# ccuchengwei/LongReadSelfCorrect

Measured on NVIDIA B200. Metric: corrected Mbp/s (seed + FM-extend + DP/MSA fallback, default options), higher is better.
Workload: dtype int64+f64

## Files before the change

### longreadselfcorrect_b200/csrc/pbsc_dp.cu

```cuda
#include <cub/cub.cuh>
#include <stdio.h>
#include <stdlib.h>
#include <string.h>
#include <algorithm>
#include <vector>
#include <type_traits>
#include "pbsc_batch.cuh"
#include "pbsc_task.cuh"
#include <chrono>
#include "pbsc_dp.cuh"
#include "pbsc_dp_thread.cuh"
#include "pbsc_dp_msa.cuh"

namespace pbsc {

constexpr int DP_HALF = 100;
constexpr int DP_BW = 2 * DP_HALF + 1;
constexpr int DP_CPL = 7;
constexpr int DP_NEG = -(1 << 28);
constexpr int DP_WARPS = 8;

struct __align__(16) DpJob
{
    uint64_t lo[4];
// ... 201 lines not shown
    }
    int bestRowVal = 0, bestRowI = 0, bestColVal = 0, bestColJ = 0;
    bool anyRow = false, anyCol = false;
    #pragma unroll 1
    for (int i = 1; i <= qlen; i++)
    {
        const int jb = origin + i;
        const int first = max(jb, 1);
        const int last = min(jb + DP_BW, nRows) - 1;
        const bool skipCol = (last + 1 <= 0) || first >= nRows || first > last;
        const int rlo = skipCol ? (1 << 20) : first - jb, rhi = skipCol ? (1 << 20) : last - jb;
        const unsigned span = skipCol ? 0u : (unsigned)(rhi - rlo);
        const int rowNoLeft = (rhi != rlo) ? rhi : -1;
        const int c1 = (int)q[i - 1];
        const int pn0 = __shfl_down_sync(FULL, prev[0], 1);
        int a[DP_CPL], cur[DP_CPL];
        int run = DP_NEG;
        #pragma unroll
        for (int t = 0; t < DP_CPL; t++)
        {
            const int r = rbase + t;
            const bool comp = (unsigned)(r - rlo) <= span;
            const int sub = sw[t] == c1 ? 1 : -8;
            const int pl = (t < DP_CPL - 1) ? prev[t + 1] : pn0;
            const int left1 = (r != rowNoLeft) ? pl - 1 : DP_NEG;
            const int v0 = __viaddmax_s32(prev[t], sub, left1);
            run = comp ? __viaddmax_s32(v0, r, run) : run;
            a[t] = run;
        }
        int incl = run;
        #pragma unroll
        for (int off = 1; off < 32; off <<= 1)
        {
            const int o = __shfl_up_sync(FULL, incl, off);
            if (lane >= off) incl = max(incl, o);
        }
        int excl = __shfl_up_sync(FULL, incl, 1);
        if (lane == 0) excl = DP_NEG;
        #pragma unroll
        for (int t = 0; t < DP_CPL; t++)
        {
            const int r = rbase + t;
            const bool comp = (unsigned)(r - rlo) <= span;
            cur[t] = comp ? max(a[t], excl) - r : idle[t];
        }
        int upPrev = __shfl_up_sync(FULL, cur[DP_CPL - 1], 1);
        if (lane == 0) upPrev = DP_NEG;
        uint32_t w = 0;
        #pragma unroll
        for (int t = 0; t < DP_CPL; t++)
        {
            const int r = rbase + t;
            const bool comp = (unsigned)(r - rlo) <= span;
            const int diag = prev[t] + (sw[t] == c1 ? 1 : -8);
            const int pl = (t < DP_CPL - 1) ? prev[t + 1] : pn0;
            const int upv = t > 0 ? cur[t - 1] : upPrev;
            uint32_t f = (cur[t] == diag) ? 1u : 0u;
            f |= (cur[t] == upv - 1) ? 2u : 0u;
            f |= (cur[t] == pl - 1) ? 4u : 0u;
            w |= (comp ? f : 0u) << (3 * t);
        }
        flags[(size_t)i * 32 + lane] = w;
        if (!skipCol && last == nRows - 1)
        {
            const int vv = __shfl_sync(FULL, incl, 31) - rhi;
            if (!anyRow || vv > bestRowVal) { bestRowVal = vv; bestRowI = i; anyRow = true; }
        }
        if (i == qlen && !skipCol)
        {
            int lv = DP_NEG, lr = 0x7fffffff;
            #pragma unroll
            for (int t = 0; t < DP_CPL; t++)
            {
                const int r = rbase + t;
                const bool comp = (unsigned)(r - rlo) <= span;
                if (comp && cur[t] > lv) { lv = cur[t]; lr = r; }
            }
            #pragma unroll
            for (int off = 16; off > 0; off >>= 1)
            {
                const int ov = __shfl_xor_sync(FULL, lv, off), orr = __shfl_xor_sync(FULL, lr, off);
                if (ov > lv || (ov == lv && orr < lr)) { lv = ov; lr = orr; }
            }
            if (lr != 0x7fffffff) { anyCol = true; bestColVal = lv; bestColJ = jb + lr; }
        }
        const int nx = __shfl_down_sync(FULL, sw[0], 1);
        #pragma unroll
        for (int t = 0; t < DP_CPL; t++) { prev[t] = cur[t]; if (t < DP_CPL - 1) sw[t] = sw[t + 1]; }
        if (lane == 31)
        {
            const int j = jb + 1 + rbase + (DP_CPL - 1);
            sw[DP_CPL - 1] = (j >= 1 && j <= mlen) ? (int)s2[j - 1] : -1;
        }
        else sw[DP_CPL - 1] = nx;
    }
    if (anyCol && (!anyRow || bestColVal > bestRowVal)) { bi = qlen; bj = bestColJ; }
    else { bi = anyRow ? bestRowI : 0; bj = nRows - 1; }
    if (!(anyRow || anyCol) || bi <= 0 || bj <= 0) bi = 0;
}

#ifndef PBSC_DP_MINB
#define PBSC_DP_MINB 2
#endif
__global__ void __launch_bounds__(DP_WARPS * 32, PBSC_DP_MINB)
dp_align_kernel(uint64_t n_rows, DpRow* rows, const DpJob* __restrict__ jobs, const WalkTask* __restrict__ tasks, uint8_t* mem, uint64_t mem0,
                uint32_t* arenas, uint64_t arena_words, unsigned long long* counter, unsigned int* n_bad)
{
    const int lane = threadIdx.x & 31;
    const int wib = threadIdx.x >> 5;
    uint32_t* arena = arenas + ((size_t)blockIdx.x * DP_WARPS + wib) * arena_words;
    for (;;)
    {
        unsigned long long base = 0;
        if (lane == 0) base = atomicAdd(counter, 32ull);
        base = __shfl_sync(FULL, base, 0);
        if (base >= n_rows) break;
        const int nb = (int)min((unsigned long long)32, n_rows - base);
        int g0 = 0;
        uint64_t used = 0;
        uint64_t my_off = 0; int my_bi = 0, my_bj = 0; bool my_todo = false;
        for (int kk = 0; kk <= nb; kk++)
        {
            uint64_t need = 0;
            DpRow R; DpJob J; RowGeom g;
            bool fill = false;
            if (kk < nb)
            {
                R = rows[base + kk];
                if (R.pass == 2)
                {
                    J = jobs[R.job];
                    row_geometry(R, J, mem, mem0, g);
                    need = ((uint64_t)g.qlen + 1) * 32;
                    fill = true;
                }
            }
            if (kk == nb || (fill && used + need > arena_words))
            {
                __syncwarp();
                if (lane >= g0 && lane < kk && my_todo)
                {
                    DpRow Rm = rows[base + lane];
                    const DpJob Jm = jobs[Rm.job];
                    RowGeom gm;
                    row_geometry(Rm, Jm, mem, mem0, gm);
                    const uint32_t* fl = arena + my_off;
                    const uint8_t* __restrict__ s2 = gm.s2;
                    const uint8_t* __restrict__ q = gm.q;
                    const int qlen = gm.qlen, mlen = gm.mlen, origin = gm.origin;
                    int i = my_bi, j = my_bj, n = 0, ed = 0;
                    if (i <= 0) { atomicAdd(n_bad, 1u); Rm.pass = 0; }
                    else
                    {
                        int r = j - (origin + i);
                        uint32_t word = fl[(size_t)i * 32 + r / DP_CPL];
                        int wcol = i, widx = r / DP_CPL;
                        #pragma unroll 1
                        while (i > 0 && j > 0)
                        {
                            r = j - (origin + i);
                            const int wi = r / DP_CPL;
                            if (wcol != i || widx != wi) { word = fl[(size_t)i * 32 + wi]; wcol = i; widx = wi; }
                            const uint32_t nextWord = i > 1 ? fl[(size_t)(i - 1) * 32 + wi] : 0u;
                            const uint32_t f = (word >> (3 * (r - wi * DP_CPL))) & 7u;
                            const int s2p = (int)s2[j - 1], s2n = j < mlen ? (int)s2[j] : -1;
                            const int s1p = (int)q[i - 1], s1n = i < qlen ? (int)q[i] : -2;
                            const bool eqD = f & 1u, eqU = (f & 2u) != 0, eqL = (f & 4u) != 0;
                            int op;
                            if (s2p == s2n) op = eqU ? OP_I : (eqL ? OP_D : OP_M);
                            else if (s1p == s1n) op = eqL ? OP_D : (eqU ? OP_I : OP_M);
                            else op = eqD ? OP_M : (eqL ? OP_D : OP_I);
                            if (op == OP_M) { if (s1p != s2p) ed++; i--; j--; }
                            else if (op == OP_I) { ed++; j--; }
                            else { ed++; i--; }
                            if (op != OP_I) { word = nextWord; wcol = i; }
                            gm.ops[n] = (uint8_t)op;
                            n++;
                        }
                        const WalkTask& tk = tasks[Jm.task];
                        const uint64_t fsum = (uint64_t)(int64_t)tk.freq_sum;
                        double identity = 0.65;
                        identity = __dadd_rn(identity, fsum > 50 ? 0.05 : 0.0);
                        identity = __dadd_rn(identity, fsum > 100 ? 0.05 : 0.0);
                        const double pct = __ddiv_rn(__dmul_rn((double)(n - ed), 100.0), (double)n);
                        const bool passOverlap = (uint64_t)n >= (uint64_t)(qlen / 10);
                        const bool passIdentity = __ddiv_rn(pct, 100.0) >= identity;
                        Rm.nops = (uint32_t)n; Rm.start0 = i; Rm.start1 = j;
                        Rm.pass = (passOverlap && passIdentity) ? 1u : 0u;
                    }
                    rows[base + lane] = Rm;
                    my_todo = false;
                }
                __syncwarp();
                g0 = kk; used = 0;
            }
            if (fill)
            {
                int bi, bj;
                dp_fill_row(g, arena + used, bi, bj);
                if (lane == kk) { my_off = used; my_bi = bi; my_bj = bj; my_todo = true; }
                used += need;
            }
        }
    }
}

template <int QMAX_, int NT_, bool GREAD_>
struct DptCfg
{
    static constexpr int QMAX = QMAX_;
    static constexpr int NT = NT_;
    static constexpr bool GREAD = GREAD_;
    static constexpr int HWORDS = dpt::HSLOTS / 2;
    static constexpr int SWORDS = (dpt::max_len_bound(QMAX_) + 15) / 16 + 1;
    static constexpr int SMEM = (HWORDS + (GREAD_ ? 0 : SWORDS)) * NT_ * 4;
};
using DptShort = DptCfg<256, 128, false>;
using DptLong = DptCfg<1024, 64, true>;
using DptHuge = DptCfg<4000, 32, true>;
constexpr uint32_t DPT_KEY_NONE = 0x3FFFu;
constexpr int DPT_KEY_BITS = 14;

__device__ __forceinline__ int dp_row_origin(const DpRow& R, const DpJob& J)
{
    const int k = (int)J.k, qlen = (int)J.qlen, mlen = (int)R.len;
    const bool isRC = R.local >= J.cnt[0] + J.cnt[1];
    const int start_1 = isRC ? qlen - k : 0, start_2 = isRC ? mlen - k : 0;
    return (start_2 - start_1 + 1) - (DP_HALF + 1);
}

__global__ void __launch_bounds__(256)
dp_keys_kernel(uint64_t n_rows, const DpRow* __restrict__ rows, const DpJob* __restrict__ jobs, uint32_t* keys, uint32_t* order, int qmax,
               unsigned long long* n_eligible)
{
    const uint64_t i = blockIdx.x * (uint64_t)blockDim.x + threadIdx.x;
    if (i >= n_rows) return;
    const DpRow R = rows[i];
    uint32_t key = DPT_KEY_NONE;
    if (R.pass == 2)
    {
        const DpJob J = jobs[R.job];
        if (dpt::eligible((int)J.qlen, (int)R.len, dp_row_origin(R, J), qmax))
            key = ((uint32_t)(qmax - (int)J.qlen) << 1) | (R.local >= J.cnt[0] + J.cnt[1] ? 1u : 0u);
    }
    keys[i] = key;
    order[i] = (uint32_t)i;
    const unsigned m = __ballot_sync(__activemask(), key != DPT_KEY_NONE);
    if (key != DPT_KEY_NONE && (threadIdx.x & 31) == __ffs(m) - 1) atomicAdd(n_eligible, (unsigned long long)__popc(m));
}

template <class C>
struct DptH
{
    uint32_t* p;
    __device__ __forceinline__ int get(int j) const
    {
        const int s = j & (dpt::HSLOTS - 1);
        return (int)reinterpret_cast<const short*>(p + (s >> 1) * C::NT)[s & 1];
    }
    __device__ __forceinline__ void set(int j, int v)
    {
        const int s = j & (dpt::HSLOTS - 1);
        reinterpret_cast<short*>(p + (s >> 1) * C::NT)[s & 1] = (short)v;
    }
    __device__ __forceinline__ bool pairs_ok(int j) const { return ((j >> 1) & (C::HWORDS - 1)) <= C::HWORDS - 5; }
    __device__ __forceinline__ uint32_t get2(int j, int u) const { return p[((j >> 1) & (C::HWORDS - 1)) * C::NT + u * C::NT]; }
    __device__ __forceinline__ void set2(int j, int u, uint32_t w) { p[((j >> 1) & (C::HWORDS - 1)) * C::NT + u * C::NT] = w; }
};
template <class C>
struct DptS
{
    const uint32_t* p;
    __device__ __forceinline__ int base(int x) const { return (int)((p[(x >> 4) * C::NT] >> (2 * (x & 15))) & 3u); }
    __device__ __forceinline__ uint32_t bits(int x) const
    {
        const uint32_t* w = p + (x >> 4) * C::NT;
        return __funnelshift_r(w[0], w[C::NT], 2 * (x & 15));
    }
};
struct DptSG
{
    const uint32_t* p;
    __device__ __forceinline__ int base(int x) const { return (int)((p[(size_t)(x >> 4) * 32] >> (2 * (x & 15))) & 3u); }
    __device__ __forceinline__ uint32_t bits(int x) const
    {
        const uint32_t* w = p + (size_t)(x >> 4) * 32;
        return __funnelshift_r(w[0], w[32], 2 * (x & 15));
    }
};
struct DptF
{
    uint32_t* p;
    __device__ __forceinline__ void put(int n, uint32_t w) { p[(size_t)n * 32] = w; }
    __device__ __forceinline__ uint32_t get(int n) const { return p[(size_t)n * 32]; }
};
struct DptQ { const uint8_t* q; __device__ __forceinline__ int operator()(int x) const { return (int)q[x]; } };
struct DptOps { uint8_t* ops; __device__ __forceinline__ void put(int n, int op) { ops[n] = (uint8_t)op; } };

template <class C>
__global__ void __launch_bounds__(C::NT, 227 * 1024 / (C::SMEM + 1024))
dp_align_thread_kernel(uint64_t n_rows, const uint32_t* __restrict__ keys, const uint32_t* __restrict__ order, DpRow* rows,
                       const DpJob* __restrict__ jobs, const WalkTask* __restrict__ tasks, uint8_t* mem, uint64_t mem0, uint32_t* arenas,
                       uint64_t arena_words, unsigned long long* counter, unsigned int* n_bad, const unsigned long long* __restrict__ n_eligible,
                       unsigned long long min_rows, unsigned int* n_thread_rows, uint32_t* rarena)
{
    extern __shared__ uint32_t dpt_smem[];
    const unsigned long long n_el = *n_eligible;
    if (n_el < min_rows) return;
    if (blockIdx.x == 0 && threadIdx.x == 0) atomicAdd(n_thread_rows, (unsigned int)n_el);
    const int lane = threadIdx.x & 31;
    uint32_t* Hs = dpt_smem + threadIdx.x;
    const uint64_t warp = (uint64_t)blockIdx.x * (C::NT / 32) + (threadIdx.x >> 5);
    uint32_t* Ss = C::GREAD ? rarena + warp * (uint64_t)(C::SWORDS * 32) + lane : dpt_smem + C::HWORDS * C::NT + threadIdx.x;
    constexpr int SSTRIDE = C::GREAD ? 32 : C::NT;
    DptF F{arenas + warp * arena_words + lane};
    for (;;)
    {
        unsigned long long base = 0;
        if (lane == 0) base = atomicAdd(counter, 32ull);
        base = __shfl_sync(FULL, base, 0);
        if (base >= n_rows) break;
        const uint64_t t = base + lane;
        const uint32_t key = t < n_rows ? keys[t] : DPT_KEY_NONE;
        if (__shfl_sync(FULL, key, 0) == DPT_KEY_NONE) break;
        if (key == DPT_KEY_NONE) continue;
        const uint64_t ri = order[t];
        DpRow R = rows[ri];
        const DpJob J = jobs[R.job];
        RowGeom g;
        row_geometry(R, J, mem, mem0, g);
        for (int x = 0; x < g.mlen; x += 16)
        {
            uint32_t w = 0;
            const int m = min(16, g.mlen - x);
            for (int y = 0; y < m; y++) w |= (uint32_t)g.s2[x + y] << (2 * y);
            Ss[(x >> 4) * SSTRIDE] = w;
        }
        Ss[((g.mlen + 15) >> 4) * SSTRIDE] = 0u;
        #pragma unroll 8
        for (int x = 0; x < C::HWORDS; x++) Hs[x * C::NT] = 0u;
        DptH<C> H{Hs};
        const typename std::conditional<C::GREAD, DptSG, DptS<C>>::type S{Ss};
        const DptQ q{g.q};
        int bi, bj;
        dpt::fill(g.qlen, g.mlen, g.origin, H, S, F, q, bi, bj);
        if (bi <= 0) { atomicAdd(n_bad, 1u); R.pass = 0; }
        else
        {
            DptOps ops{g.ops};
            int n, ed, i0, j0;
            dpt::traceback(g.qlen, g.mlen, g.origin, S, F, q, bi, bj, ops, n, ed, i0, j0);
            const WalkTask& tk = tasks[J.task];
            const uint64_t fsum = (uint64_t)(int64_t)tk.freq_sum;
            double identity = 0.65;
            identity = __dadd_rn(identity, fsum > 50 ? 0.05 : 0.0);
            identity = __dadd_rn(identity, fsum > 100 ? 0.05 : 0.0);
            const double pct = __ddiv_rn(__dmul_rn((double)(n - ed), 100.0), (double)n);
            const bool passOverlap = (uint64_t)n >= (uint64_t)(g.qlen / 10);
            const bool passIdentity = __ddiv_rn(pct, 100.0) >= identity;
            R.nops = (uint32_t)n; R.start0 = i0; R.start1 = j0;
            R.pass = (passOverlap && passIdentity) ? 1u : 0u;
        }
        rows[ri] = R;
    }
}

struct MsaCtx
{
    WalkTask& tk; uint8_t* outpool;
    __device__ __forceinline__ int min_call() const
    {
        const uint64_t fsum = (uint64_t)(int64_t)tk.freq_sum;
        return (int)(fsum > 50 ? (uint64_t)__dmul_rn((double)fsum, 0.4) : 15);
    }
    __device__ __forceinline__ uint8_t* out() const { return outpool + tk.out_off; }
    __device__ __forceinline__ uint32_t cap() const { return tk.out_cap; }
};

__global__ void __launch_bounds__(128)
dp_job_keys_kernel(uint64_t j0, uint64_t j1, const DpJob* __restrict__ jobs, const DpRow* __restrict__ rows, uint64_t row_base, uint32_t* keys,
                   uint32_t* order)
{
    const uint64_t t = blockIdx.x * (uint64_t)blockDim.x + threadIdx.x;
    if (j0 + t >= j1) return;
    const DpJob J = jobs[j0 + t];
    const uint32_t nr = job_rows_of(J);
    const DpRow* R = rows + (J.row0 - row_base);
    uint32_t passing = 0, cost = 0;
    for (uint32_t r = 0; r < nr; r++)
    {
        const DpRow x = R[r];
        if (x.pass == 1) { passing++; cost += x.nops; }
    }
    if (passing < 3) cost = 0;
    keys[t] = 0xFFFFu - min(0xFFFFu, cost >> 3);
    order[t] = (uint32_t)t;
}

__global__ void __launch_bounds__(64)
dp_msa_kernel(uint64_t j0, uint64_t j1, const uint32_t* __restrict__ order, int deal, const DpJob* __restrict__ jobs, WalkTask* tasks,
              const DpRow* __restrict__ rows, uint64_t row_base, uint8_t* mem, uint64_t mem0, uint8_t* outpool, unsigned int* n_bad,
              uint32_t big_thr, uint32_t* big_list, unsigned int* n_big)
{
    const uint64_t tx = blockIdx.x * (uint64_t)blockDim.x + threadIdx.x;
    const uint64_t njc = j1 - j0;
    uint64_t rank = tx;
    if (order && deal)
    {
        const uint64_t n_warps = (njc + 31) / 32;
        rank = (tx & 31) * n_warps + (tx >> 5);
        if (tx >= n_warps * 32) return;
    }
    if (rank >= njc) return;
    const uint64_t jx = j0 + (order ? order[rank] : rank);
    const DpJob J = jobs[jx];
    WalkTask& tk = tasks[J.task];
    const uint32_t nr = job_rows_of(J);
    const DpRow* R = rows + (J.row0 - row_base);
    if (big_list)
    {
        uint32_t cost = 0, passing = 0;
        for (uint32_t r = 0; r < nr; r++) { const DpRow x = R[r]; if (x.pass == 1) { passing++; cost += x.nops; } }
        if (passing >= 3 && cost >= big_thr) { big_list[atomicAdd(n_big, 1u)] = (uint32_t)(jx - j0); return; }
    }
    JobView v;
    job_view(mem + (J.mem - mem0), J, nr, v);
    const MsaCtx ctx{tk, outpool};
    uint32_t n = 0;
    const int rc = msa::consensus(v, J.qlen, J.k, R, nr, ctx, n);
    if (rc == 1) { tk.dp_status = PBSC_DP_FEW_ROWS; return; }
    if (rc == 2) { atomicAdd(n_bad, 1u); tk.dp_status = PBSC_OVF_DP; return; }
    tk.out_len = n;
    tk.dp_status = PBSC_DP_OK;
}

constexpr int MSA_WARPS = 4;
__global__ void __launch_bounds__(MSA_WARPS * 32)
dp_msa_warp_kernel(uint64_t j0, const uint32_t* __restrict__ big_list, const unsigned int* __restrict__ n_big, unsigned long long* counter,
                   const DpJob* __restrict__ jobs, WalkTask* tasks, const DpRow* __restrict__ rows, uint64_t row_base, uint8_t* mem, uint64_t mem0,
                   uint8_t* outpool, unsigned int* n_bad)
{
    __shared__ unsigned int gap_counter[MSA_WARPS];
    const int lane = threadIdx.x & 31, warp = threadIdx.x >> 5;
    const unsigned long long n = *n_big;
    for (;;)
    {
        unsigned long long it = 0;
        if (lane == 0) it = atomicAdd(counter, 1ull);
        it = __shfl_sync(0xffffffffu, it, 0);
        if (it >= n) break;
        const uint64_t jx = j0 + big_list[it];
        const DpJob J = jobs[jx];
        WalkTask& tk = tasks[J.task];
        const uint32_t nr = job_rows_of(J);
        const DpRow* R = rows + (J.row0 - row_base);
        JobView v;
        job_view(mem + (J.mem - mem0), J, nr, v);
        const MsaCtx ctx{tk, outpool};
        uint32_t nout = 0;
        const int rc = msa::consensus_warp(v, J.qlen, J.k, R, nr, ctx, nout, &gap_counter[warp]);
        __syncwarp();
        if (lane == 0)
        {
            if (rc == 1) tk.dp_status = PBSC_DP_FEW_ROWS;
            else if (rc == 2) { atomicAdd(n_bad, 1u); tk.dp_status = PBSC_OVF_DP; }
            else { tk.out_len = nout; tk.dp_status = PBSC_DP_OK; }
        }
        __syncwarp();
    }
}

template <class T>
static cudaError_t arena(pbsc_index* idx, const char* name, size_t count, T** out) { return arena_get(idx, name, (count ? count : 1) * sizeof(T), (void**)out); }

DpStats& last_dp_stats() { static thread_local DpStats s; return s; }

struct DptPass
{
    bool on = false; uint64_t qmax = 0, arena_words = 0, min_rows = 0, read_words = 0; int blocks = 0;
    uint64_t flag_words() const { return on ? arena_words * (uint64_t)blocks : 0; }
};
template <class C>
static cudaError_t dpt_pass_setup(pbsc_index* idx, uint64_t q_longest, uint64_t q_prev_max, int cap_per_sm, DptPass& g)
{
    g.on = q_longest > q_prev_max;
    if (!g.on) return cudaSuccess;
    g.qmax = std::min<uint64_t>((uint64_t)C::QMAX, q_longest);
    g.arena_words = 32ull * g.qmax * dpt::WMAX;
    cudaError_t e = cudaFuncSetAttribute(dp_align_thread_kernel<C>, cudaFuncAttributeMaxDynamicSharedMemorySize, C::SMEM);
    if (e != cudaSuccess) return e;
    int per = 0;
    e = cudaOccupancyMaxActiveBlocksPerMultiprocessor(&per, dp_align_thread_kernel<C>, C::NT, C::SMEM);
    if (e != cudaSuccess) return e;
    if (cap_per_sm > 0) per = std::min(per, cap_per_sm);
    g.blocks = idx->sm_count * std::max(per, 1);
    g.arena_words *= (uint64_t)(C::NT / 32);
    g.read_words = C::GREAD ? (uint64_t)g.blocks * (C::NT / 32) * (uint64_t)(C::SWORDS * 32) : 0;
    return cudaSuccess;
}
template <class C>
static void dpt_pass_launch(const DptPass& g, cudaStream_t st, uint64_t nrows, DpRow* rows, const DpJob* jobs, const WalkTask* tasks, uint8_t* mem,
                            uint64_t mem0, uint32_t* keys, uint32_t* keys2, uint32_t* order, uint32_t* order2, uint8_t* sort_tmp, size_t sort_bytes,
                            uint32_t* slabs, unsigned long long* counter, unsigned int* cnt, uint32_t* rarena)
{
    cudaMemsetAsync(counter, 0, 16, st);
    dp_keys_kernel<<<(unsigned)((nrows + 255) / 256), 256, 0, st>>>(nrows, rows, jobs, keys, order, (int)g.qmax, counter + 1);
    cub::DeviceRadixSort::SortPairs(sort_tmp, sort_bytes, keys, keys2, order, order2, (int)nrows, 0, DPT_KEY_BITS, st);
    const int tb = (int)std::min<uint64_t>((uint64_t)g.blocks, (nrows + C::NT - 1) / C::NT);
    dp_align_thread_kernel<C><<<tb, C::NT, C::SMEM, st>>>(nrows, keys2, order2, rows, jobs, tasks, mem, mem0, slabs, g.arena_words / (C::NT / 32), counter,
                                                          cnt + 1, counter + 1, g.min_rows, cnt + 2, rarena);
}

int run_dp_fallback(pbsc_index* idx, const pbsc_params* p, DeviceBatch& b, void* tasks_v, uint64_t n_items, const uint32_t* list, uint8_t* outpool,
                    uint32_t q_cap, uint64_t* launches)
{
    WalkTask* tasks = (WalkTask*)tasks_v;
    cudaStream_t st = idx->stream;
    if (n_items == 0) return PBSC_OK;
    const bool htrace = getenv("PBSC_ROUND_TRACE") != nullptr;
    auto h0 = std::chrono::steady_clock::now();
    auto hmark = [&](const char* what) {
        if (!htrace) return;
        const auto now = std::chrono::steady_clock::now();
        const double ms = std::chrono::duration<double, std::milli>(now - h0).count();
        if (ms > 2.0) fprintf(stderr, "[pbsc round trace]     dp host: %-22s %8.2f ms\n", what, ms);
        h0 = now;
    };
    DpJob* jobs; uint64_t *job_rows, *job_bytes, *row_off, *mem_off; unsigned int* cnt; unsigned long long* qctr;
    PBSC_CUDA(arena(idx, "dp.jobs", n_items, &jobs));
    PBSC_CUDA(arena(idx, "dp.job_rows", n_items + 1, &job_rows));
    PBSC_CUDA(arena(idx, "dp.job_bytes", n_items + 1, &job_bytes));
    PBSC_CUDA(arena(idx, "dp.row_off", n_items + 1, &row_off));
    PBSC_CUDA(arena(idx, "dp.mem_off", n_items + 1, &mem_off));
    PBSC_CUDA(arena(idx, "dp.cnt", 4, &cnt));
    PBSC_CUDA(arena(idx, "dp.qctr", 4, &qctr));
    PBSC_CUDA(cudaMemsetAsync(cnt, 0, 16, st));
    cudaEvent_t ev[2];
    PBSC_CUDA(cudaEventCreate(&ev[0])); PBSC_CUDA(cudaEventCreate(&ev[1]));
    struct EvGuard { cudaEvent_t* e; ~EvGuard() { cudaEventDestroy(e[0]); cudaEventDestroy(e[1]); } } guard{ev};
    PBSC_CUDA(cudaEventRecord(ev[0], st));
    dp_collect_kernel<<<(unsigned)((n_items + 127) / 128), 128, 0, st>>>(idx->dev, n_items, list, tasks, b.codes.p, b.offsets.p, (uint32_t)p->pb_coverage,
                                                                        jobs, job_rows, job_bytes, cnt);
    unsigned int hcnt[4] = {0, 0, 0, 0};
    PBSC_CUDA(cudaMemcpyAsync(hcnt, cnt, 16, cudaMemcpyDeviceToHost, st));
    PBSC_CUDA(cudaStreamSynchronize(st));
    if (launches) *launches += 1;
    const uint64_t nj = hcnt[0];
    DpStats& S = last_dp_stats();
    hmark("collect + sync");
    if (nj == 0) return PBSC_OK;
    {
        size_t tb = 0, tb2 = 0;
        cub::DeviceScan::ExclusiveSum(nullptr, tb, job_rows, row_off, (int)(nj + 1), st);
        cub::DeviceScan::ExclusiveSum(nullptr, tb2, job_bytes, mem_off, (int)(nj + 1), st);
        tb = std::max(tb, tb2);
        uint8_t* tmp;
        PBSC_CUDA(arena(idx, "dp.cubtmp", tb, &tmp));
        PBSC_CUDA(cudaMemsetAsync(job_rows + nj, 0, 8, st));
        PBSC_CUDA(cudaMemsetAsync(job_bytes + nj, 0, 8, st));
        cub::DeviceScan::ExclusiveSum(tmp, tb, job_rows, row_off, (int)(nj + 1), st);
        cub::DeviceScan::ExclusiveSum(tmp, tb, job_bytes, mem_off, (int)(nj + 1), st);
        dp_offsets_kernel<<<(unsigned)((nj + 255) / 256), 256, 0, st>>>(nj, jobs, row_off, mem_off);
    }
    std::vector<uint64_t> h_row(nj + 1), h_mem(nj + 1);
    PBSC_CUDA(cudaMemcpyAsync(h_row.data(), row_off, (nj + 1) * 8, cudaMemcpyDeviceToHost, st));
    PBSC_CUDA(cudaMemcpyAsync(h_mem.data(), mem_off, (nj + 1) * 8, cudaMemcpyDeviceToHost, st));
    PBSC_CUDA(cudaStreamSynchronize(st));
    if (launches) *launches += 3;
    hmark("scans + sync");
    S.jobs += nj; S.rows += h_row[nj];
    uint64_t budget = 20ull << 30;
    {
        const auto it = idx->arena.find("dp.mem");
        const uint64_t have = it != idx->arena.end() ? (uint64_t)it->second.cap : 0;
        if (h_mem[nj] > have)
        {
            size_t free_b = 0, total_b = 0;
            if (cudaMemGetInfo(&free_b, &total_b) == cudaSuccess) budget = std::min<uint64_t>(budget, std::max<uint64_t>(2ull << 30, (free_b + have) / 2));
        }
        else budget = std::max<uint64_t>(have, 1);
    }
    if (const char* e = getenv("PBSC_DP_CHUNK_MB")) { if (atoll(e) > 0) budget = (uint64_t)atoll(e) << 20; }
    uint64_t max_job = 0;
    for (uint64_t j = 0; j < nj; j++) max_job = std::max(max_job, h_mem[j + 1] - h_mem[j]);
    if (max_job > budget) budget = max_job;
    const uint64_t pool_bytes = std::min(budget, h_mem[nj]);
    uint8_t* mem;
    hmark("budget");
    PBSC_CUDA(arena(idx, "dp.mem", pool_bytes, &mem));
    hmark("arena dp.mem");
    int per_sm = 0;
    PBSC_CUDA(cudaOccupancyMaxActiveBlocksPerMultiprocessor(&per_sm, dp_align_kernel, DP_WARPS * 32, 0));
    if (per_sm < 1) per_sm = 1;
    if (const char* e = getenv("PBSC_DP_BLOCKS_PER_SM")) { if (atoi(e) > 0) per_sm = std::min(per_sm, atoi(e)); }
    const int ablocks = idx->sm_count * per_sm;
    uint64_t arena_words = std::max<uint64_t>(((uint64_t)q_cap + 2) * 32, 1ull << 18);
    if (const char* e = getenv("PBSC_DP_ARENA_KB")) { if (atoll(e) > 0) arena_words = std::max<uint64_t>(((uint64_t)q_cap + 2) * 32, (uint64_t)atoll(e) * 256); }
    uint32_t* slabs;
    PBSC_CUDA(arena(idx, "dp.flags", arena_words * (uint64_t)ablocks * DP_WARPS, &slabs));
    uint64_t max_rows = 0;
    for (uint64_t j0 = 0; j0 < nj;)
    {
        uint64_t j1 = j0 + 1;
        while (j1 < nj && h_mem[j1 + 1] - h_mem[j0] <= pool_bytes) j1++;
        max_rows = std::max(max_rows, h_row[j1] - h_row[j0]);
        j0 = j1;
    }
    DpRow* rows;
    hmark("flags arena + chunking");
    PBSC_CUDA(arena(idx, "dp.rows", max_rows, &rows));
    bool use_thread = true;
    if (const char* e = getenv("PBSC_DP_THREAD")) use_thread = atoi(e) != 0;
    uint32_t *tkeys = nullptr, *tkeys2 = nullptr, *torder = nullptr, *torder2 = nullptr, *tslabs = nullptr, *treads = nullptr;
    uint8_t* sort_tmp = nullptr;
    size_t sort_bytes = 0;
    const uint64_t q_longest = std::min<uint64_t>(q_cap, hcnt[3]);
    DptPass pass_s, pass_l, pass_h;
    if (use_thread)
    {
        int cap = 0;
        if (const char* e = getenv("PBSC_DPT_BLOCKS_PER_SM")) cap = atoi(e);
        const bool longer = !(getenv("PBSC_DPT_LONG") && atoi(getenv("PBSC_DPT_LONG")) == 0);
        PBSC_CUDA(dpt_pass_setup<DptShort>(idx, q_longest, 0, cap, pass_s));
        if (longer) PBSC_CUDA(dpt_pass_setup<DptLong>(idx, q_longest, DptShort::QMAX, 0, pass_l));
        if (longer) PBSC_CUDA(dpt_pass_setup<DptHuge>(idx, q_longest, DptLong::QMAX, 0, pass_h));
        pass_s.min_rows = 512; pass_l.min_rows = 2048; pass_h.min_rows = 2048;
        if (const char* e = getenv("PBSC_DPT_MIN_ROWS")) pass_s.min_rows = pass_l.min_rows = pass_h.min_rows = (uint64_t)std::max(0ll, atoll(e));
        PBSC_CUDA(arena(idx, "dp.tkeys", max_rows, &tkeys));
        PBSC_CUDA(arena(idx, "dp.tkeys2", max_rows, &tkeys2));
        PBSC_CUDA(arena(idx, "dp.torder", max_rows, &torder));
        PBSC_CUDA(arena(idx, "dp.torder2", max_rows, &torder2));
        cub::DeviceRadixSort::SortPairs(nullptr, sort_bytes, tkeys, tkeys2, torder, torder2, (int)max_rows, 0, DPT_KEY_BITS, st);
        PBSC_CUDA(arena(idx, "dp.sorttmp", sort_bytes, &sort_tmp));
        PBSC_CUDA(arena(idx, "dp.tflags", std::max(pass_s.flag_words(), std::max(pass_l.flag_words(), pass_h.flag_words())), &tslabs));
        PBSC_CUDA(arena(idx, "dp.treads", std::max<uint64_t>(1, std::max(pass_l.on ? pass_l.read_words : 0, pass_h.on ? pass_h.read_words : 0)), &treads));
    }
    int sort_jobs = 0;
    if (const char* e = getenv("PBSC_DP_SORT_JOBS")) sort_jobs = atoi(e);
    uint32_t *jkeys = nullptr, *jkeys2 = nullptr, *jord = nullptr, *jord2 = nullptr;
    uint8_t* jsort_tmp = nullptr;
    size_t jsort_bytes = 0;
    if (sort_jobs)
    {
        PBSC_CUDA(arena(idx, "dp.jkeys", nj, &jkeys));
        PBSC_CUDA(arena(idx, "dp.jkeys2", nj, &jkeys2));
        PBSC_CUDA(arena(idx, "dp.jord", nj, &jord));
        PBSC_CUDA(arena(idx, "dp.jord2", nj, &jord2));
        cub::DeviceRadixSort::SortPairs(nullptr, jsort_bytes, jkeys, jkeys2, jord, jord2, (int)nj, 0, 16, st);
        PBSC_CUDA(arena(idx, "dp.jsorttmp", jsort_bytes, &jsort_tmp));
    }
    uint32_t msa_big_thr = 8192;
    if (const char* e = getenv("PBSC_MSA_WARP_MIN")) msa_big_thr = atoll(e) < 0 ? 0xffffffffu : (uint32_t)atoll(e);
    uint32_t* msa_big = nullptr;
    unsigned long long* msa_q = nullptr;
    PBSC_CUDA(arena(idx, "dp.msa_big", nj, &msa_big));
    PBSC_CUDA(arena(idx, "dp.msa_q", 2, &msa_q));
    struct Prof
    {
        bool on = false; cudaStream_t st; std::vector<std::pair<const char*, cudaEvent_t>> ev;
        void mark(const char* name) { if (!on) return; cudaEvent_t e; cudaEventCreate(&e); cudaEventRecord(e, st); ev.emplace_back(name, e); }
        void report()
        {
            if (!on || ev.size() < 2) return;
            cudaEventSynchronize(ev.back().second);
            std::vector<std::pair<const char*, float>> acc;
            for (size_t x = 1; x < ev.size(); x++)
            {
                float ms = 0; cudaEventElapsedTime(&ms, ev[x - 1].second, ev[x].second);
                bool found = false;
                for (auto& a : acc) if (!strcmp(a.first, ev[x].first)) { a.second += ms; found = true; }
                if (!found) acc.emplace_back(ev[x].first, ms);
            }
            fprintf(stderr, "[pbsc dp profile]");
            for (auto& a : acc) fprintf(stderr, " %s %.1f ms;", a.first, a.second);
            fprintf(stderr, "\n");
            for (auto& e : ev) cudaEventDestroy(e.second);
        }
    } prof;
    prof.st = st;
    if (const char* e = getenv("PBSC_DP_PROFILE")) prof.on = atoi(e) != 0;
    hmark("pass setup + arenas");
    prof.mark("start");
    for (uint64_t j0 = 0; j0 < nj;)
    {
        uint64_t j1 = j0 + 1;
        while (j1 < nj && h_mem[j1 + 1] - h_mem[j0] <= pool_bytes) j1++;
        const uint64_t nrows = h_row[j1] - h_row[j0], njc = j1 - j0;
        dp_rows_kernel<<<(unsigned)((njc + 127) / 128), 128, 0, st>>>(j0, j1, jobs, tasks, b.codes.p, b.offsets.p, mem, h_mem[j0], rows, h_row[j0]);
        dp_retrieve_kernel<<<(unsigned)((nrows + 127) / 128), 128, 0, st>>>(idx->dev, nrows, rows, jobs, mem, h_mem[j0]);
        prof.mark("rows+retrieve");
        PBSC_CUDA(cudaMemsetAsync(qctr, 0, 32, st));
        if (pass_s.on)
        {
            dpt_pass_launch<DptShort>(pass_s, st, nrows, rows, jobs, tasks, mem, h_mem[j0], tkeys, tkeys2, torder, torder2, sort_tmp, sort_bytes, tslabs,
                                      qctr + 1, cnt, treads);
            prof.mark("align_thread_256");
            if (launches) *launches += 4;
        }
        if (pass_l.on)
        {
            dpt_pass_launch<DptLong>(pass_l, st, nrows, rows, jobs, tasks, mem, h_mem[j0], tkeys, tkeys2, torder, torder2, sort_tmp, sort_bytes, tslabs,
                                     qctr + 1, cnt, treads);
            prof.mark("align_thread_1024");
            if (launches) *launches += 4;
        }
        if (pass_h.on)
        {
            dpt_pass_launch<DptHuge>(pass_h, st, nrows, rows, jobs, tasks, mem, h_mem[j0], tkeys, tkeys2, torder, torder2, sort_tmp, sort_bytes, tslabs,
                                     qctr + 1, cnt, treads);
            prof.mark("align_thread_4000");
            if (launches) *launches += 4;
        }
        const int nb = (int)std::min<uint64_t>((uint64_t)ablocks, (nrows + DP_WARPS * 32 - 1) / (DP_WARPS * 32));
        dp_align_kernel<<<nb, DP_WARPS * 32, 0, st>>>(nrows, rows, jobs, tasks, mem, h_mem[j0], slabs, arena_words, qctr, cnt + 1);
        prof.mark("align_warp");
        const uint32_t* jorder = nullptr;
        if (sort_jobs)
        {
            dp_job_keys_kernel<<<(unsigned)((njc + 127) / 128), 128, 0, st>>>(j0, j1, jobs, rows, h_row[j0], jkeys, jord);
            size_t sb = jsort_bytes;
            cub::DeviceRadixSort::SortPairs(jsort_tmp, sb, jkeys, jkeys2, jord, jord2, (int)njc, 0, 16, st);
            jorder = jord2;
            if (launches) *launches += 3;
        }
        PBSC_CUDA(cudaMemsetAsync(msa_q, 0, 16, st));
        dp_msa_kernel<<<(unsigned)((((njc + 31) / 32) * 32 + 63) / 64), 64, 0, st>>>(j0, j1, jorder, sort_jobs == 1, jobs, tasks, rows, h_row[j0], mem,
                                                                                         h_mem[j0], outpool, cnt + 1, msa_big_thr,
                                                                                         msa_big_thr != 0xffffffffu ? msa_big : nullptr, (unsigned int*)(msa_q + 1));
        prof.mark("msa");
        if (msa_big_thr != 0xffffffffu)
        {
            const int wb = (int)std::min<uint64_t>((uint64_t)idx->sm_count * 4, (njc + MSA_WARPS - 1) / MSA_WARPS);
            dp_msa_warp_kernel<<<wb, MSA_WARPS * 32, 0, st>>>(j0, msa_big, (const unsigned int*)(msa_q + 1), msa_q, jobs, tasks, rows, h_row[j0], mem, h_mem[j0],
                                                              outpool, cnt + 1);
            prof.mark("msa_warp");
            if (launches) *launches += 1;
        }
        PBSC_CUDA(cudaGetLastError());
        if (launches) *launches += 4;
        S.chunks++;
        j0 = j1;
    }
    PBSC_CUDA(cudaEventRecord(ev[1], st));
    hmark("chunk loop (launches)");
    prof.report();
    PBSC_CUDA(cudaMemcpyAsync(hcnt, cnt, 12, cudaMemcpyDeviceToHost, st));
    PBSC_CUDA(cudaStreamSynchronize(st));
    S.bad += hcnt[1];
    S.thread_rows += hcnt[2];
    PBSC_OCC_TAKE(3, st);
    float ms = 0;
    cudaEventElapsedTime(&ms, ev[0], ev[1]);
    S.ms += ms;
    return PBSC_OK;
}

}
```

### longreadselfcorrect_b200/csrc/pbsc_dp_thread.cuh

```cuda
#ifndef PBSC_DP_THREAD_CUH
#define PBSC_DP_THREAD_CUH

#include <stdint.h>

#if defined(__CUDACC__)
#define PBSC_DPT_HD __host__ __device__ __forceinline__
#else
#define PBSC_DPT_HD inline
#endif

namespace pbsc { namespace dpt {

constexpr int HALF = 100;
constexpr int BW = 2 * HALF + 1;
constexpr int CPW = 10;
constexpr int WMAX = (BW + CPW - 1) / CPW;
constexpr int NEVER = -(1 << 28);
constexpr int OP_M = 0, OP_I = 1, OP_D = 2;
constexpr int HSLOTS = 256;

PBSC_DPT_HD uint32_t push_ne(uint32_t w, int v, int x)
{
#if defined(__CUDA_ARCH__)
    return __funnelshift_l((uint32_t)(x - v), w, 1);
#else
    return (w << 1) | ((uint32_t)(x - v) >> 31);
#endif
}
PBSC_DPT_HD int imax(int a, int b) { return a > b ? a : b; }
PBSC_DPT_HD int imin(int a, int b) { return a < b ? a : b; }

PBSC_DPT_HD constexpr int max_len_bound(int qmax) { return qmax + qmax / 10 + 21; }

PBSC_DPT_HD bool eligible(int qlen, int mlen, int , int qmax) { return qlen >= 1 && qlen <= qmax && mlen >= 1 && mlen <= max_len_bound(qmax); }
PBSC_DPT_HD int words_per_col(int mlen) { return (imin(BW, mlen) + 1 + CPW - 1) / CPW; }

template <class HS, class SS, class FS, class QF>
PBSC_DPT_HD void fill(int qlen, int mlen, int origin, HS& H, const SS& S, FS& F, const QF& q, int& bi, int& bj)
{
    const int nRows = mlen + 1;
    const int W = words_per_col(mlen);
    int bestRowVal = 0, bestRowI = 0;
    bool anyRow = false;
    int wbase = 0;
#if defined(__CUDA_ARCH__)
    #pragma unroll 1
#endif
    for (int i = 1; i <= qlen; i++, wbase += W)
    {
        const int jb = origin + i;
        const int first = imax(jb, 1);
        const int last = imin(jb + BW, nRows) - 1;
        if (last < first) continue;
        const int c1 = q(i - 1);
        const uint32_t c1rep = (uint32_t)c1 * 0x55555u;
        int j = first;
        int diagOld = H.get(j - 1);
        int widx = wbase, kin = (first & 1) + 1;
        int up, v;
        uint32_t w;
        {
            const int leftOld = H.get(j);
            const int d = diagOld + (S.base(j - 1) == c1 ? 1 : -8);
            const int l1 = (j == jb + BW - 1) ? NEVER : leftOld - 1;
            const int u1 = first > jb ? -1 : NEVER;
            v = imax(d, l1);
            w = (v == d ? 1u : 0u) | (v == u1 ? 2u : 0u) | (v == l1 ? 4u : 0u);
            H.set(j, v);
            up = v; diagOld = leftOld;
            j++;
        }
        auto rolled = [&](int jend)
        {
#if defined(__CUDA_ARCH__)
            #pragma unroll 1
#endif
            for (; j < jend; j++)
            {
                const int leftOld = H.get(j);
                const int d = diagOld + (S.base(j - 1) == c1 ? 1 : -8);
                const int l1 = leftOld - 1, u1 = up - 1;
                const int vv = imax(imax(d, l1), u1);
                w = (w << 3) | (vv == d ? 1u : 0u) | (vv == u1 ? 2u : 0u) | (vv == l1 ? 4u : 0u);
                H.set(j, vv);
                up = vv; diagOld = leftOld;
                if (++kin == CPW) { F.put(widx++, w); w = 0; kin = 0; }
            }
        };
        rolled(imin(last, (first & ~1) + CPW));
#if defined(__CUDA_ARCH__)
        #pragma unroll 1
#endif
        while (j + CPW <= last)
        {
            if (!H.pairs_ok(j)) { rolled(j + CPW); continue; }
            const uint32_t x = S.bits(j - 1) ^ c1rep;
            uint32_t ww = 0;
#if defined(__CUDA_ARCH__)
            #pragma unroll
#endif
            for (int u = 0; u < CPW / 2; u++)
            {
                const uint32_t old2 = H.get2(j, u);
                const int leftA = (int)(int16_t)(old2 & 0xFFFFu), leftB = (int)old2 >> 16;
                const int eA = diagOld + ((x & (3u << (4 * u))) == 0u ? 2 : -7);
                const int xA = imax(imax(eA, leftA), up);
                const int vA = xA - 1;
                const int eB = leftA + ((x & (12u << (4 * u))) == 0u ? 2 : -7);
                const int xB = imax(imax(eB, leftB), vA);
                const int vB = xB - 1;
                ww = push_ne(push_ne(push_ne(ww, xA, leftA), xA, up), xA, eA);
                ww = push_ne(push_ne(push_ne(ww, xB, leftB), xB, vA), xB, eB);
                H.set2(j, u, ((uint32_t)vA & 0xFFFFu) | ((uint32_t)vB << 16));
                up = vB; diagOld = leftB;
            }
            F.put(widx++, ww ^ 0x3FFFFFFFu);
            j += CPW;
        }
        rolled(last);
        if (last > first)
        {
            const int d = diagOld + (S.base(last - 1) == c1 ? 1 : -8);
            const int u1 = up - 1;
            const int l1 = (last == jb + BW - 1) ? NEVER : H.get(last) - 1;
            v = imax(d, u1);
            w = (w << 3) | (v == d ? 1u : 0u) | (v == u1 ? 2u : 0u) | (v == l1 ? 4u : 0u);
            H.set(last, v);
            if (++kin == CPW) { F.put(widx++, w); w = 0; kin = 0; }
        }
        if (kin) F.put(widx, w << (3 * (CPW - kin)));
        if (last == nRows - 1 && (!anyRow || v > bestRowVal)) { bestRowVal = v; bestRowI = i; anyRow = true; }
    }
    int bestColVal = 0, bestColJ = 0;
    bool anyCol = false;
    {
        const int jb = origin + qlen;
        const int first = imax(jb, 1), last = imin(jb + BW, nRows) - 1;
        for (int j = first; j <= last; j++)
        {
            const int v = H.get(j);
            if (!anyCol || v > bestColVal) { bestColVal = v; bestColJ = j; anyCol = true; }
        }
    }
    if (anyCol && (!anyRow || bestColVal > bestRowVal)) { bi = qlen; bj = bestColJ; }
    else { bi = anyRow ? bestRowI : 0; bj = nRows - 1; }
    if (!(anyRow || anyCol) || bi <= 0 || bj <= 0) bi = 0;
}

template <class SS, class FS, class QF, class OS>
PBSC_DPT_HD void traceback(int qlen, int mlen, int origin, const SS& S, const FS& F, const QF& q, int bi, int bj, OS& ops,
                           int& n_out, int& ed_out, int& i_out, int& j_out)
{
    const int W = words_per_col(mlen);
    int i = bi, j = bj, n = 0, ed = 0;
    int ckey = -1;
    uint32_t cword = 0;
#if defined(__CUDA_ARCH__)
    #pragma unroll 1
#endif
    while (i > 0 && j > 0)
    {
        const int k = j - (imax(origin + i, 1) & ~1);
        const int kw = k / CPW;
        const int key = (i - 1) * W + kw;
        if (key != ckey) { cword = F.get(key); ckey = key; }
        const uint32_t f = (cword >> (3 * (CPW - 1 - (k - kw * CPW)))) & 7u;
        const int s2p = S.base(j - 1), s2n = j < mlen ? S.base(j) : -1;
        const int s1p = q(i - 1), s1n = i < qlen ? q(i) : -2;
        const bool eqD = (f & 1u) != 0, eqU = (f & 2u) != 0, eqL = (f & 4u) != 0;
        int op;
        if (s2p == s2n) op = eqU ? OP_I : (eqL ? OP_D : OP_M);
        else if (s1p == s1n) op = eqL ? OP_D : (eqU ? OP_I : OP_M);
        else op = eqD ? OP_M : (eqL ? OP_D : OP_I);
        if (op == OP_M) { if (s1p != s2p) ed++; i--; j--; }
        else if (op == OP_I) { ed++; j--; }
        else { ed++; i--; }
        ops.put(n, op);
        n++;
    }
    n_out = n; ed_out = ed; i_out = i; j_out = j;
}

}}

#endif
```

Baseline: 81.86.

## Fill two DP columns at once with packed 16-bit SIMD lanes

Adds a paired-column fill path to the per-thread banded DP that computes two adjacent query columns together, packing both into 16-bit halves and using __vadd2, __vimax3_s16x2, __viaddmax_s16x2 and byte_perm for the recurrence and traceback flags. The aim is to halve the H-row shared-memory reads and writes and roughly halve instruction count per cell in the fill loop, which dominates thread-level DP alignment. It is on by default and can be disabled with PBSC_DPT_PAIR. The risks are 16-bit overflow, which the host emulation checks but the device does not, more complex edge-case handling at band boundaries, and higher register pressure.

```diff
diff --git a/longreadselfcorrect_b200/csrc/pbsc_dp.cu b/longreadselfcorrect_b200/csrc/pbsc_dp.cu
--- a/longreadselfcorrect_b200/csrc/pbsc_dp.cu
+++ b/longreadselfcorrect_b200/csrc/pbsc_dp.cu
@@ -527,7 +527,7 @@
 dp_align_thread_kernel(uint64_t n_rows, const uint32_t* __restrict__ keys, const uint32_t* __restrict__ order, DpRow* rows,
                        const DpJob* __restrict__ jobs, const WalkTask* __restrict__ tasks, uint8_t* mem, uint64_t mem0, uint32_t* arenas,
                        uint64_t arena_words, unsigned long long* counter, unsigned int* n_bad, const unsigned long long* __restrict__ n_eligible,
-                       unsigned long long min_rows, unsigned int* n_thread_rows, uint32_t* rarena)
+                       unsigned long long min_rows, unsigned int* n_thread_rows, uint32_t* rarena, int pair)
 {
     extern __shared__ uint32_t dpt_smem[];
     const unsigned long long n_el = *n_eligible;
@@ -568,7 +568,7 @@
         const typename std::conditional<C::GREAD, DptSG, DptS<C>>::type S{Ss};
         const DptQ q{g.q};
         int bi, bj;
-        dpt::fill(g.qlen, g.mlen, g.origin, H, S, F, q, bi, bj);
+        dpt::fill(g.qlen, g.mlen, g.origin, H, S, F, q, bi, bj, pair != 0);
         if (bi <= 0) { atomicAdd(n_bad, 1u); R.pass = 0; }
         else
         {
@@ -703,6 +703,7 @@
 struct DptPass
 {
     bool on = false; uint64_t qmax = 0, arena_words = 0, min_rows = 0, read_words = 0; int blocks = 0;
+    int pair = 1;
     uint64_t flag_words() const { return on ? arena_words * (uint64_t)blocks : 0; }
 };
 template <class C>
@@ -733,7 +734,7 @@
     cub::DeviceRadixSort::SortPairs(sort_tmp, sort_bytes, keys, keys2, order, order2, (int)nrows, 0, DPT_KEY_BITS, st);
     const int tb = (int)std::min<uint64_t>((uint64_t)g.blocks, (nrows + C::NT - 1) / C::NT);
     dp_align_thread_kernel<C><<<tb, C::NT, C::SMEM, st>>>(nrows, keys2, order2, rows, jobs, tasks, mem, mem0, slabs, g.arena_words / (C::NT / 32), counter,
-                                                          cnt + 1, counter + 1, g.min_rows, cnt + 2, rarena);
+                                                          cnt + 1, counter + 1, g.min_rows, cnt + 2, rarena, g.pair);
 }
 
 int run_dp_fallback(pbsc_index* idx, const pbsc_params* p, DeviceBatch& b, void* tasks_v, uint64_t n_items, const uint32_t* list, uint8_t* outpool,
@@ -851,6 +852,7 @@
         if (longer) PBSC_CUDA(dpt_pass_setup<DptHuge>(idx, q_longest, DptLong::QMAX, 0, pass_h));
         pass_s.min_rows = 512; pass_l.min_rows = 2048; pass_h.min_rows = 2048;
         if (const char* e = getenv("PBSC_DPT_MIN_ROWS")) pass_s.min_rows = pass_l.min_rows = pass_h.min_rows = (uint64_t)std::max(0ll, atoll(e));
+        if (const char* e = getenv("PBSC_DPT_PAIR")) pass_s.pair = pass_l.pair = pass_h.pair = atoi(e) != 0 ? 1 : 0;
         PBSC_CUDA(arena(idx, "dp.tkeys", max_rows, &tkeys));
         PBSC_CUDA(arena(idx, "dp.tkeys2", max_rows, &tkeys2));
         PBSC_CUDA(arena(idx, "dp.torder", max_rows, &torder));
diff --git a/longreadselfcorrect_b200/csrc/pbsc_dp_thread.cuh b/longreadselfcorrect_b200/csrc/pbsc_dp_thread.cuh
--- a/longreadselfcorrect_b200/csrc/pbsc_dp_thread.cuh
+++ b/longreadselfcorrect_b200/csrc/pbsc_dp_thread.cuh
@@ -2,6 +2,8 @@
 #define PBSC_DP_THREAD_CUH
 
 #include <stdint.h>
+#include <stdio.h>
+#include <stdlib.h>
 
 #if defined(__CUDACC__)
 #define PBSC_DPT_HD __host__ __device__ __forceinline__
@@ -35,23 +37,74 @@
 PBSC_DPT_HD bool eligible(int qlen, int mlen, int , int qmax) { return qlen >= 1 && qlen <= qmax && mlen >= 1 && mlen <= max_len_bound(qmax); }
 PBSC_DPT_HD int words_per_col(int mlen) { return (imin(BW, mlen) + 1 + CPW - 1) / CPW; }
 
+#if !defined(__CUDA_ARCH__)
+PBSC_DPT_HD int lo16(uint32_t x) { return (int)(int16_t)(x & 0xFFFFu); }
+PBSC_DPT_HD int hi16(uint32_t x) { return (int)(int16_t)(x >> 16); }
+PBSC_DPT_HD uint32_t pk16(int lo, int hi)
+{
+    if (lo < -32768 || lo > 32767 || hi < -32768 || hi > 32767) { printf("packed 16-bit lane overflow\n"); abort(); }
+    return (uint32_t)(uint16_t)lo | ((uint32_t)(uint16_t)hi << 16);
+}
+#endif
+PBSC_DPT_HD uint32_t v2add(uint32_t a, uint32_t b)
+{
+#if defined(__CUDA_ARCH__)
+    return __vadd2(a, b);
+#else
+    return pk16(lo16(a) + lo16(b), hi16(a) + hi16(b));
+#endif
+}
+PBSC_DPT_HD uint32_t v2sub(uint32_t a, uint32_t b)
+{
+#if defined(__CUDA_ARCH__)
+    return __vsub2(a, b);
+#else
+    return pk16(lo16(a) - lo16(b), hi16(a) - hi16(b));
+#endif
+}
+PBSC_DPT_HD uint32_t v2max3(uint32_t a, uint32_t b, uint32_t c)
+{
+#if defined(__CUDA_ARCH__)
+    return __vimax3_s16x2(a, b, c);
+#else
+    return pk16(imax(imax(lo16(a), lo16(b)), lo16(c)), imax(imax(hi16(a), hi16(b)), hi16(c)));
+#endif
+}
+PBSC_DPT_HD uint32_t v2addmax(uint32_t a, uint32_t b, uint32_t c)
+{
+#if defined(__CUDA_ARCH__)
+    return __viaddmax_s16x2(a, b, c);
+#else
+    return pk16(imax(lo16(a) + lo16(b), lo16(c)), imax(hi16(a) + hi16(b), hi16(c)));
+#endif
+}
+PBSC_DPT_HD uint32_t prmt(uint32_t a, uint32_t b, uint32_t sel)
+{
+#if defined(__CUDA_ARCH__)
+    return __byte_perm(a, b, sel);
+#else
+    const uint64_t ab = (uint64_t)a | ((uint64_t)b << 32);
+    uint32_t r = 0;
+    for (int k = 0; k < 4; k++) r |= (uint32_t)((ab >> (8 * ((sel >> (4 * k)) & 7u))) & 0xFFu) << (8 * k);
+    return r;
+#endif
+}
+
+struct FillBest { int rowVal = 0, rowI = 0; bool anyRow = false; };
+PBSC_DPT_HD void note_last_row(FillBest& b, int v, int i)
+{
+    if (!b.anyRow || v > b.rowVal) { b.rowVal = v; b.rowI = i; b.anyRow = true; }
+}
+
 template <class HS, class SS, class FS, class QF>
-PBSC_DPT_HD void fill(int qlen, int mlen, int origin, HS& H, const SS& S, FS& F, const QF& q, int& bi, int& bj)
+PBSC_DPT_HD void fill_col(int i, int mlen, int origin, int wbase, HS& H, const SS& S, FS& F, const QF& q, FillBest& best)
 {
     const int nRows = mlen + 1;
-    const int W = words_per_col(mlen);
-    int bestRowVal = 0, bestRowI = 0;
-    bool anyRow = false;
-    int wbase = 0;
-#if defined(__CUDA_ARCH__)
-    #pragma unroll 1
-#endif
-    for (int i = 1; i <= qlen; i++, wbase += W)
     {
         const int jb = origin + i;
         const int first = imax(jb, 1);
         const int last = imin(jb + BW, nRows) - 1;
-        if (last < first) continue;
+        if (last < first) return;
         const int c1 = q(i - 1);
         const uint32_t c1rep = (uint32_t)c1 * 0x55555u;
         int j = first;
@@ -129,8 +182,193 @@
             if (++kin == CPW) { F.put(widx++, w); w = 0; kin = 0; }
         }
         if (kin) F.put(widx, w << (3 * (CPW - kin)));
-        if (last == nRows - 1 && (!anyRow || v > bestRowVal)) { bestRowVal = v; bestRowI = i; anyRow = true; }
+        if (last == nRows - 1) note_last_row(best, v, i);
     }
+}
+
+PBSC_DPT_HD bool pairable(int i, int mlen, int origin)
+{
+    const int jb = origin + i;
+    return jb <= 0 ? jb + BW - 1 >= 1 : (jb >= 2 && (jb & 1) == 0 && jb + 1 <= mlen);
+}
+
+template <class HS, class SS, class FS, class QF>
+PBSC_DPT_HD void fill_pair(int i, int mlen, int origin, int wbase, HS& H, const SS& S, FS& F, const QF& q, FillBest& best)
+{
+    const int nRows = mlen + 1;
+    const int W = words_per_col(mlen);
+    const int jbA = origin + i, jbB = jbA + 1;
+    const int fA = imax(jbA, 1), fB = imax(jbB, 1);
+    const int lA = imin(jbA + BW, nRows) - 1, lB = imin(jbB + BW, nRows) - 1;
+    const int cA = q(i - 1), cB = q(i);
+    const uint32_t cArep = (uint32_t)cA * 0x55555u, cBrep = (uint32_t)cB * 0x55555u;
+    int hA = H.get(fA - 1), a1 = 0, a2 = 0, b1 = 0;
+    uint32_t wA = 0, wB = 0;
+    int kA = 0, kB = 0, xA = wbase, xB = wbase + W;
+    int vAl = 0, vBl = 0;
+    int sx0 = fA - 1;
+    uint32_t sw0 = S.bits(sx0), sw1 = 0;
+    auto sbase = [&](int x)
+    {
+        const int d = x - sx0;
+        return (int)((d < CPW ? sw0 >> (2 * d) : sw1 >> (2 * (d - CPW))) & 3u);
+    };
+    auto step = [&](int j)
+    {
+        int aj = a1;
+        if (j <= lA)
+        {
+            const int left = H.get(j);
+            const int d = hA + (sbase(j - 1) == cA ? 1 : -8);
+            const int l1 = (j == jbA + BW - 1) ? NEVER : left - 1;
+            int v;
+            uint32_t f;
+            if (j == fA)
+            {
+                const int u1 = fA > jbA ? -1 : NEVER;
+                v = imax(d, l1);
+                f = (v == d ? 1u : 0u) | (v == u1 ? 2u : 0u) | (v == l1 ? 4u : 0u);
+                wA = f; kA = (fA & 1) + 1;
+            }
+            else
+            {
+                const int u1 = a1 - 1;
+                v = j == lA ? imax(d, u1) : imax(imax(d, l1), u1);
+                f = (v == d ? 1u : 0u) | (v == u1 ? 2u : 0u) | (v == l1 ? 4u : 0u);
+                wA = (wA << 3) | f;
+                if (++kA == CPW) { F.put(xA++, wA); wA = 0; kA = 0; }
+            }
+            if (j == lA) vAl = v;
+            hA = left; aj = v;
+        }
+        const int r = j - 1;
+        if (r >= fB && r <= lB)
+        {
+            const int d = a2 + (sbase(r - 1) == cB ? 1 : -8);
+            const int l1 = (r == jbB + BW - 1) ? NEVER : a1 - 1;
+            int v;
+            uint32_t f;
+            if (r == fB)
+            {
+                const int u1 = fB > jbB ? -1 : NEVER;
+                v = imax(d, l1);
+                f = (v == d ? 1u : 0u) | (v == u1 ? 2u : 0u) | (v == l1 ? 4u : 0u);
+                wB = f; kB = (fB & 1) + 1;
+            }
+            else
+            {
+                const int u1 = b1 - 1;
+                v = r == lB ? imax(d, u1) : imax(imax(d, l1), u1);
+                f = (v == d ? 1u : 0u) | (v == u1 ? 2u : 0u) | (v == l1 ? 4u : 0u);
+                wB = (wB << 3) | f;
+                if (++kB == CPW) { F.put(xB++, wB); wB = 0; kB = 0; }
+            }
+            H.set(r, v);
+            if (r == lB) vBl = v;
+            b1 = v;
+        }
+        a2 = a1; a1 = aj;
+    };
+    int j = fA;
+    const int jw = (fA & ~1) + CPW;
+#if defined(__CUDA_ARCH__)
+    #pragma unroll 1
+#endif
+    for (; j < jw; j++) step(j);
+#if defined(__CUDA_ARCH__)
+    #pragma unroll 1
+#endif
+    if (j + CPW <= lA)
+    {
+#if defined(__CUDA_ARCH__)
+        uint32_t D = (uint32_t)(hA & 0xFFFF) | ((uint32_t)a2 << 16), V = (uint32_t)(a1 & 0xFFFF) | ((uint32_t)b1 << 16);
+#else
+        uint32_t D = pk16(hA, a2), V = pk16(a1, b1);
+#endif
+        uint32_t na = S.bits(j - 1), nb = S.bits(j - 2);
+#if defined(__CUDA_ARCH__)
+        #pragma unroll 1
+#endif
+        do
+        {
+            const uint32_t xa = na ^ cArep, xb = nb ^ cBrep;
+            if (j + 2 * CPW <= lA) { na = S.bits(j + CPW - 1); nb = S.bits(j + CPW - 2); }
+            const uint32_t ma = (xa | (xa >> 1)) & 0x55555u, mb = (xb | (xb >> 1)) & 0x55555u;
+            const uint32_t m1 = (ma & 0xFFFFu) | (mb << 16);
+            const uint32_t m2 = (ma >> 16) | (mb & 0xF0000u);
+            uint32_t hw[CPW / 2];
+#if defined(__CUDA_ARCH__)
+            #pragma unroll
+#endif
+            for (int u = 0; u < CPW / 2; u++) hw[u] = H.get2(j + 2 * u, 0);
+            uint32_t Wa = 0, Wb = 0;
+#if defined(__CUDA_ARCH__)
+            #pragma unroll
+#endif
+            for (int s = 0; s < CPW; s++)
+            {
+                const uint32_t p = (s < 8 ? m1 >> (2 * s) : m2 >> (2 * (s - 8))) & 0x00010001u;
+                const uint32_t e = v2add(D, p * 0xFFF7u + 0x00020002u);
+                const uint32_t L = prmt(hw[s >> 1], V, (s & 1) ? 0x5432u : 0x5410u);
+                const uint32_t X = v2max3(e, L, V);
+                const uint32_t K = v2add(~X, 0x00030003u);
+                const uint32_t f = v2addmax(e, K, 0x00010001u) + (v2addmax(V, K, 0x00010001u) << 1) + (v2addmax(L, K, 0x00010001u) << 2);
+                if (s < CPW / 2) Wa = (Wa << 3) + f; else Wb = (Wb << 3) + f;
+                const uint32_t Vn = v2add(X, 0xFFFFFFFFu);
+                if ((s & 1) == 0) H.set2(j + s - 2, 0, prmt(V, Vn, 0x7632u));
+                D = L; V = Vn;
+            }
+            Wa -= 0x7FFF7FFFu; Wb -= 0x7FFF7FFFu;
+            F.put(xA++, ((Wa & 0x7FFFu) << 15) | (Wb & 0x7FFFu));
+            F.put(xB++, (wB << 3) | (Wa >> 28));
+            wB = ((Wa >> 1) & 0x7FF8000u) | (Wb >> 16);
+            j += CPW;
+        } while (j + CPW <= lA);
+#if defined(__CUDA_ARCH__)
+        hA = (int)(short)(D & 0xFFFFu); a2 = (int)D >> 16; a1 = (int)(short)(V & 0xFFFFu); b1 = (int)V >> 16;
+#else
+        hA = lo16(D); a2 = hi16(D); a1 = lo16(V); b1 = hi16(V);
+#endif
+        H.set(j - 2, b1);
+    }
+    sx0 = j - 2;
+    sw0 = sx0 <= mlen - 1 ? S.bits(sx0) : 0u;
+    sw1 = sx0 + CPW <= imin(lA, mlen - 1) ? S.bits(sx0 + CPW) : 0u;
+#if defined(__CUDA_ARCH__)
+    #pragma unroll 1
+#endif
+    for (; j <= lB + 1; j++) step(j);
+    if (kA) F.put(xA, wA << (3 * (CPW - kA)));
+    if (kB) F.put(xB, wB << (3 * (CPW - kB)));
+    if (lA == nRows - 1) note_last_row(best, vAl, i);
+    if (lB == nRows - 1) note_last_row(best, vBl, i + 1);
+}
+
+template <class HS, class SS, class FS, class QF>
+PBSC_DPT_HD void fill(int qlen, int mlen, int origin, HS& H, const SS& S, FS& F, const QF& q, int& bi, int& bj, bool pair = true)
+{
+    const int nRows = mlen + 1;
+    const int W = words_per_col(mlen);
+    FillBest best;
+    int i = 1, wbase = 0;
+#if defined(__CUDA_ARCH__)
+    #pragma unroll 1
+#endif
+    while (i <= qlen)
+    {
+        if (pair && i < qlen && pairable(i, mlen, origin))
+        {
+            fill_pair(i, mlen, origin, wbase, H, S, F, q, best);
+            i += 2; wbase += 2 * W;
+        }
+        else
+        {
+            fill_col(i, mlen, origin, wbase, H, S, F, q, best);
+            i++; wbase += W;
+        }
+    }
+    const int bestRowVal = best.rowVal, bestRowI = best.rowI;
+    const bool anyRow = best.anyRow;
     int bestColVal = 0, bestColJ = 0;
     bool anyCol = false;
     {
```

Result: faster. 87.21, median of 6 (+6.5%).
